# dmMaze/comic-text-detector

Hardware: AMD Instinct MI355X
Metric: pages/sec at 1024x1024 bs=32 (end-to-end detector, device-resident pages) (higher is better)
Workload: dtype f16

## Files before the change

### comic-text-detector_amd/_lib.py

```python
from __future__ import annotations

import ctypes as C
import os
import subprocess

_HERE = os.path.dirname(os.path.abspath(__file__))
LIB_PATH = os.path.join(_HERE, "libctd_hip.so")
SELFTEST_PATH = os.path.join(_HERE, "ctd_selftest")

ABI_VERSION = 8
OK = 0
PREC_F32, PREC_F16, PREC_F32S = 0, 1, 2
ACT = {"none": 0, "silu": 1, "leaky": 2, "relu": 3, "sigmoid": 4}
IN_NCHW_F32, IN_NHWC_U8 = 0, 1
(OP_INPUT, OP_CONV, OP_CONVT, OP_MAXPOOL, OP_AVGPOOL2, OP_DETECT, OP_EXPORT, OP_STEM, OP_SEG_FINAL,
 OP_DB_UP) = range(1, 11)
OUT_MASK, OUT_LINES = 0, 1
REGION_OK, REGION_DEGENERATE, REGION_MAX_SIDE, REGION_TILE = 0, 1, 32766, 1024
REGION_U8, REGION_F16, REGION_F32 = 0, 1, 2
LAYOUT_NCHW, LAYOUT_NHWC = 0, 1


class CtdTensor(C.Structure):
    _fields_ = [("channels", C.c_int32), ("log2_down", C.c_int32), ("dtype", C.c_int32)]
# ... 64 lines not shown
    "ctd_ccl_workspace_bytes": (C.c_size_t, [_i32, _i32, _i32]),
    "ctd_ccl": (_i32, [_vp, _i32, _i32, _i32, _i32, _i32, _vp, _vp, _vp, _i32, _vp, C.c_size_t, _vp]),
    "ctd_ccl_dual": (_i32, [_vp, _i32, _i32, _i32, _i32, _vp, _vp, _vp, _vp, _vp, _vp, _vp, _i32, _vp, C.c_size_t, _vp]),
    "ctd_resize_linear_u8": (_i32, [_vp, _i32, _i32, _i32, _vp, _i32, _i32, _i32, _i32, _vp]),
    "ctd_region_transforms": (_i32, [_vp, _vp, _vp, _vp, _vp, _vp, _i32, C.c_double, _vp, _vp, _vp, _vp]),
    "ctd_warp_regions": (_i32, [_vp, _i32, _vp, _i32, _vp, _vp]),
    "ctd_warp_region_batches": (_i32, [_vp, _i32, _vp, _i32, _vp, _vp, _i32, _i32, _i32, _i32, _vp]),
    "ctd_db_boxes": (_i32, [_vp, _vp, _vp, _i32, _vp, _vp, _i32, _i32, _i32, _i32, C.c_double, _vp, _vp, C.POINTER(_i32)]),
    "ctd_tail_create": (_i32, [C.POINTER(_vp), _i32]),
    "ctd_tail_destroy": (None, [_vp]),
    "ctd_tail_stream": (_vp, [_vp]),
    "ctd_tail_run": (_i32, [_vp, _i32, _i32, _i32, _vp, _i32, _i32, _vp, _vp, _i64, _vp, C.POINTER(CtdTailPage),
                            C.POINTER(CtdTailParams), _vp, _vp, _vp]),
    "ctd_tail_timings": (_i32, [_vp, C.POINTER(C.c_double)]),
    "ctd_tail_refine_paths": (_i32, [_vp, C.POINTER(_i32)]),
    "ctd_tail_db_boxes": (_i32, [_vp, _i32, _i32, _i32, _vp, _i64, _vp, _i32, C.c_double]),
    "ctd_tail_refine": (_i32, [_vp, _i32, C.POINTER(CtdTailPage), _vp, _vp, _vp, _i32, _i32, _vp, _vp]),
    "ctd_tail_page_counts": (_i32, [_vp, _i32, C.POINTER(_i32), C.POINTER(_i32), C.POINTER(_i32), C.POINTER(_i32),
                                    C.POINTER(_i32)]),
    "ctd_tail_page_fetch": (_i32, [_vp, _i32, _vp, _vp, _vp, _vp, _vp, _vp, _vp, _vp]),
    "ctd_tail_batch_counts": (_i32, [_vp, _vp]),
    "ctd_tail_batch_fetch": (_i32, [_vp, _vp, _vp, _vp]),
    "ctd_tail_pack_records": (_i32, [_vp, _i32, _i32, _vp]),
    "ctd_tail_set_threads": (_i32, [_vp, _i32]),
    "ctd_db_boxes_compact": (_i32, [_i32, _i32, _i32, _vp, _vp, _vp, _vp, _vp, _i32, _vp, _vp, _vp, _vp, _vp, _vp, _vp, _vp,
                                    _vp, _i32, C.c_double, _vp, _vp, C.POINTER(_i32)]),
    "ctd_topk_colors": (_i32, [_vp, _vp]),
    "ctd_otsu_from_hist": (_i32, [_vp]),
    "ctd_inrange_bounds": (None, [C.c_double, C.c_double, C.POINTER(_i32), C.POINTER(_i32)]),
    "ctd_group_output": (_i32, [_vp, _vp, _i32, _vp, _i32, _i32, _i32, _vp, _i32, _vp, _i32, _vp, _i32, _vp, _i32,
# ... 70 lines not shown
```

### comic-text-detector_amd/csrc/engine.hip

```cpp
#include <algorithm>
#include <cmath>
#include <cstdio>
#include <cstdlib>
#include <cstring>
#include <string>
#include <vector>

#include "kernels.h"

namespace {

thread_local std::string g_err;

int fail(int code, const std::string& msg) {
  g_err = msg;
  return code;
}

#define HIP_TRY(expr)                                                                              \
  do {                                                                                             \
    hipError_t _e = (expr);                                                                        \
    if (_e != hipSuccess)                                                                          \
      return fail(CTD_ERR_HIP, std::string(#expr) + ": " + hipGetErrorString(_e));                 \
  } while (0)
// ... 1023 lines not shown
}

int ctd_fail_msg(int code, const std::string& msg) { return fail(code, msg); }
extern int g_tail_priority;
extern int g_tail_cus, g_tail_cu_first;
extern long long g_tail_dma_min;
#ifdef CTD_MEASURE_KNOBS
extern int g_tail_skip_pages;
extern int g_tail_ablate;
#endif
extern int g_tail_chain;
extern int g_tail_fused_rounds;
extern long long g_tail_fused_max_pix;
extern int g_tail_lds, g_tail_lds_rcap, g_tw_lds_runs_x10, g_tw_lds_threads;
extern long long g_tail_lds_cls0, g_tail_lds_cls1;
extern long long g_tail_lds_max_bytes;

extern "C" {

const char* ctd_last_error(void) { return g_err.c_str(); }
int32_t ctd_abi_version(void) { return CTD_ABI_VERSION; }

int ctd_device_info(int32_t device, char* name, int32_t* cu_count, int64_t* hbm_bytes) {
  hipDeviceProp_t p;
  HIP_TRY(hipGetDeviceProperties(&p, device));
  if (name) { std::strncpy(name, p.name, 255); name[255] = 0; }
  if (cu_count) *cu_count = p.multiProcessorCount;
  if (hbm_bytes) *hbm_bytes = (int64_t)p.totalGlobalMem;
  int arch = 0;
  const char* g = std::strstr(p.gcnArchName, "gfx");
// ... 145 lines not shown
int ctd_tuning_set(const char* key, int64_t value) {
  const std::string k = key ? key : "";
  if (k == "fuse") g_fuse = (int)value;
  else if (k == "tail_max_blocks") g_tail_max_blocks = (int)std::max<int64_t>(1, value);
  else if (k == "tail_chain") g_tail_chain = (int)value;
  else if (k == "tail_fused_rounds") g_tail_fused_rounds = (int)value;
  else if (k == "tail_fused_max_pix") g_tail_fused_max_pix = value;
  else if (k == "tail_lds") g_tail_lds = (int)value;
  else if (k == "tail_lds_rcap") g_tail_lds_rcap = (int)value;
  else if (k == "tail_lds_max_bytes") g_tail_lds_max_bytes = value;
  else if (k == "tail_lds_runs_x10") g_tw_lds_runs_x10 = (int)std::max<int64_t>(1, value);
  else if (k == "tail_lds_threads") g_tw_lds_threads = (int)value;
  else if (k == "tail_lds_cls0") g_tail_lds_cls0 = value;
  else if (k == "tail_lds_cls1") g_tail_lds_cls1 = value;
  else if (k == "tail_dma_min") g_tail_dma_min = value;
#ifdef CTD_MEASURE_KNOBS
  else if (k == "tail_skip_page_download") g_tail_skip_pages = value != 0;
  else if (k == "tail_ablate") g_tail_ablate = (int)value;
#endif
  else if (k == "tail_priority") g_tail_priority = (int)value;
  else if (k == "tail_cus") g_tail_cus = (int)value;
  else if (k == "tail_cu_first") g_tail_cu_first = (int)value;
  else if (k == "no_reuse") g_no_reuse = (int)value;
  else if (k == "f32_mfma") g_f32_mfma = (int)value;
  else if (k == "split_halo") g_split_halo = (int)value;
  else if (k == "split_halo_min_patches") g_split_halo_min_patches = value;
  else if (k == "fwd_prio") g_fwd_prio = (int)value;
  else if (k == "split_stem") g_split_stem = (int)value;
  else if (k == "split_planes") g_split_planes = (int)value;
  else if (k == "db_up_mfma") g_db_up_mfma = (int)value;
// ... 101 lines not shown
```

### comic-text-detector_amd/csrc/tail.h

```cpp
#pragma once
#include "ctd_common.h"

extern int g_tail_max_blocks;

struct DbcTables {
  int B, H, W, cap, rcap;
  const float* prob;
  long long prob_stride;
  const int* lab;
  const int* n_f;
  const int* n_b;
  const int* st_f;
  const int* st_b;
  const int* first_f;
  const int* first_b;
  int* par_f;
  int* par_b;
  int* off_f;
  int* off_b;
  int* hdr;
  int* row_lo;
  int* row_hi;
  double* sum_f;
  double* sum_b;
  double* ring_sum;
  int* ring_cnt;
};
void launch_dbc(const DbcTables& t, hipStream_t st);

struct TWin {
  const uint8_t* img;
  const uint8_t* mask;
  uint8_t* out;
  int img_w, mask_w, out_w;
  int x1, y1, w, h;
  int mx, my;
  int band0, nband;
};
struct TRule {
  int kind;
  int lo, hi;
};
struct TBand {
// ... 49 lines not shown
```

### comic-text-detector_amd/csrc/tail.hip

```cpp
#include <algorithm>
#include <atomic>
#include <chrono>
#include <mutex>
#include <cmath>
#include <cstring>
#include <string>
#include <thread>
#include <vector>

#include "host_refine.h"
#include "kernels.h"
#include "tail.h"

int ctd_fail_msg(int code, const std::string& msg);
int g_tail_priority = 1;
int g_tail_cus = 0, g_tail_cu_first = 0;

#define T_TRY(expr)                                                                                  \
  do {                                                                                               \
    hipError_t e_ = (expr);                                                                          \
    if (e_ != hipSuccess) return ctd_fail_msg(CTD_ERR_HIP, std::string(#expr) + ": " + hipGetErrorString(e_)); \
  } while (0)

namespace {
// ... 82 lines not shown
  auto work = [&]() {
    for (int i; (i = next.fetch_add(1)) < n;) f(i);
  };
  std::vector<std::thread> th;
  th.reserve(nt - 1);
  for (int k = 1; k < nt; ++k) th.emplace_back(work);
  work();
  for (auto& x : th) x.join();
}

}
int g_tail_chain = 1;
int g_tail_fused_rounds = 1;
long long g_tail_fused_max_pix = 100000;
int g_tail_lds = 1, g_tail_lds_rcap = 0;
long long g_tail_lds_max_bytes = 150 << 10;
long long g_tail_lds_cls0 = 40 << 10, g_tail_lds_cls1 = 80 << 10;
namespace {
struct ChainState {
  std::mutex mu;
  hipEvent_t last = nullptr;
  hipEvent_t ring[16] = {};
  unsigned next = 0;
};
constexpr int kChainDevices = 64;
inline ChainState* chain_state(int device) {
  static ChainState states[kChainDevices];
  return device >= 0 && device < kChainDevices ? &states[device] : nullptr;
}
struct GpuChain {
// ... 81 lines not shown
  if (a.type == hipMemoryTypeHost && a.devicePointer) return a.devicePointer;
  return nullptr;
}

inline double now_ms() {
  return std::chrono::duration<double, std::milli>(std::chrono::steady_clock::now().time_since_epoch()).count();
}

}

struct ctd_tail {
  int device = 0;
  hipStream_t st = nullptr;
  DevBuf d_dets, d_nms_ws, d_lab_f, d_ccl_ws, d_ccl_small, d_dbc_i, d_dbc_d, d_rows, d_pmask, d_refined;
  DevBuf d_wins, d_rules, d_bands, d_hist, d_sums, d_canvas, d_clab, d_cstats, d_cnt, d_merged, d_mlab, d_mstats, d_cnt2, d_small, d_crop;
  DevBuf d_wins_c, d_bands_c, d_lds;
  PinBuf h_dets, h_hdr, h_tab, h_pmask, h_refined, h_hist, h_sums, h_wins, h_rules, h_bands, h_small, h_lab;
  PinBuf h_wins_c, h_bands_c, h_lds;
  int B = 0;
  std::vector<ctd_tail_page> pages;
  std::vector<size_t> poff;
  std::vector<uint8_t*> hmask;
  size_t ptotal = 0;
  std::vector<PageOut> out;
  double ms_stage[10] = {0, 0, 0, 0, 0, 0, 0, 0, 0, 0};
  double ms_db_wait = 0;
  double ms_sub[5] = {0, 0, 0, 0, 0};
  int host_threads = 8;
  int n_lds = 0, n_canvas = 0, n_ovf = 0;
  long long lds_per_block = 64 << 10;
  double ms_lds_wait = 0;
};

namespace {

struct Packed {
  std::vector<int> x, y;
  int W = 0, H = 0;
};
void shelf_pack(const std::vector<int>& w, const std::vector<int>& h, int min_width, Packed& out) {
  const int n = (int)w.size();
  out.x.assign(n, 0);
  out.y.assign(n, 0);
  int cw = min_width;
// ... 392 lines not shown
  const double w0 = now_ms();
  T_TRY(hipStreamSynchronize(st));
  t->ms_sub[3] = now_ms() - w0;
  return CTD_OK;
}

struct DbStage {
  int B = 0, Hn = 0, Wn = 0;
  const float* prob = nullptr;
  long long prob_stride = 0;
  int *lab = nullptr, *n_f = nullptr, *n_b = nullptr, *st_f = nullptr, *st_b = nullptr;
  int *first_f = nullptr, *first_b = nullptr, *par_f = nullptr, *par_b = nullptr, *off_f = nullptr, *off_b = nullptr;
  int *hdr = nullptr, *ring_cnt = nullptr, *row_lo = nullptr, *row_hi = nullptr;
  double *sum_f = nullptr, *sum_b = nullptr, *ring_sum = nullptr;
  int* hhdr = nullptr;
};

int db_enqueue(ctd_tail* t, DbStage& d, int B, int Hn, int Wn, const float* prob_dev, long long prob_stride,
               const uint8_t* bitmap_dev, Batch& pre, Batch& post) {
  hipStream_t st = t->st;
  const size_t hw = (size_t)Hn * Wn;
  const int cap = kCompCap, rcap = kRowCap;
  d.B = B, d.Hn = Hn, d.Wn = Wn, d.prob = prob_dev, d.prob_stride = prob_stride;
  GET(t->d_lab_f, (size_t)B * hw * 4, int, lab);
  GET(t->d_ccl_ws, ccl_workspace_bytes(B, Hn, Wn), uint8_t, ccl_ws);
  const size_t bc = (size_t)B * cap;
  GET(t->d_dbc_i, (2 * (size_t)B + 10 * bc + 6 * bc + 4 * (size_t)B + bc) * 4, int, ti);
  d.lab = lab;
  d.n_f = ti;
  d.n_b = d.n_f + B;
  d.st_f = d.n_b + B;
  d.st_b = d.st_f + 5 * bc;
  d.first_f = d.st_b + 5 * bc;
  d.first_b = d.first_f + bc;
  d.par_f = d.first_b + bc;
  d.par_b = d.par_f + bc;
  d.off_f = d.par_b + bc;
  d.off_b = d.off_f + bc;
  d.hdr = d.off_b + bc;
  d.ring_cnt = d.hdr + 4 * (size_t)B;
  GET(t->d_dbc_d, 3 * bc * 8, double, td);
  d.sum_f = td, d.sum_b = td + bc, d.ring_sum = td + 2 * bc;
  GET(t->d_rows, 2 * (size_t)B * rcap * 4, int, rows);
  d.row_lo = rows, d.row_hi = rows + (size_t)B * rcap;
  pre.fill(td, 0, 3 * bc * 8);
  pre.fill(d.ring_cnt, 0, bc * 4);
  pre.flush();
  launch_ccl_dual(bitmap_dev, B, Hn, Wn, 0, lab, d.n_f, d.n_b, d.st_f, d.st_b, d.first_f, d.first_b, cap, ccl_ws, st);
  DbcTables dt;
  dt.B = B, dt.H = Hn, dt.W = Wn, dt.cap = cap, dt.rcap = rcap;
  dt.prob = prob_dev, dt.prob_stride = prob_stride;
  dt.lab = lab, dt.n_f = d.n_f, dt.n_b = d.n_b, dt.st_f = d.st_f, dt.st_b = d.st_b;
  dt.first_f = d.first_f, dt.first_b = d.first_b, dt.par_f = d.par_f, dt.par_b = d.par_b, dt.off_f = d.off_f;
  dt.off_b = d.off_b, dt.hdr = d.hdr, dt.row_lo = d.row_lo, dt.row_hi = d.row_hi, dt.sum_f = d.sum_f, dt.sum_b = d.sum_b;
  dt.ring_sum = d.ring_sum, dt.ring_cnt = d.ring_cnt;
  launch_dbc(dt, st);
  GET(t->h_hdr, (size_t)B * 4 * 4, int, hhdr);
  d.hhdr = hhdr;
  T_TRY(post.d2h(hhdr, d.hdr, (size_t)B * 16));
// ... 71 lines not shown
    int nbox = 0;
    const int rc = ctd_db_boxes_compact(Wn, Hn, hhdr[4 * b], h_st_f + (size_t)b * nf * 5, h_first_f + (size_t)b * nf,
                                        h_par_f + (size_t)b * nf, h_off_f + (size_t)b * nf, h_sum_f + (size_t)b * nf,
                                        hhdr[4 * b + 1], h_st_b + (size_t)b * nb * 5, h_first_b + (size_t)b * nb,
                                        h_par_b + (size_t)b * nb, h_off_b + (size_t)b * nb, h_sum_b + (size_t)b * nb,
                                        h_ring_sum + (size_t)b * nb, h_ring_cnt + (size_t)b * nb, h_row_lo + (size_t)b * nr,
                                        h_row_hi + (size_t)b * nr, maxc, prm->unclip_ratio, po.db_boxes.data(),
                                        po.db_scores.data(), &nbox);
    if (rc) err = rc;
    po.db_boxes.resize((size_t)nbox * 8);
    po.db_scores.resize(nbox);
  });
  if (err) return ctd_fail_msg(err, "ctd_db_boxes_compact failed");
  std::vector<int16_t> boxes((size_t)std::max(maxc, 1) * 8);
  std::vector<float> scores((size_t)std::max(maxc, 1));
  for (int b = 0; b < B; ++b) {
    if (!hhdr[4 * b + 3]) continue;
    PageOut& po = t->out[b];
    int nbox = 0;
    {
      std::vector<int32_t> lab_host_f(hw), lab_host_b(hw);
      std::vector<float> prob_h(hw);
      int nfb[2];
      T_TRY(hipMemcpyAsync(nfb, d.n_f + b, 4, hipMemcpyDeviceToHost, st));
      T_TRY(hipMemcpyAsync(nfb + 1, d.n_b + b, 4, hipMemcpyDeviceToHost, st));
      T_TRY(hipMemcpyAsync(lab_host_f.data(), d.lab + (size_t)b * hw, hw * 4, hipMemcpyDeviceToHost, st));
      T_TRY(hipMemcpyAsync(prob_h.data(), d.prob + (size_t)b * d.prob_stride, hw * 4, hipMemcpyDeviceToHost, st));
      T_TRY(hipStreamSynchronize(st));
      for (size_t i = 0; i < hw; ++i) {
        const int32_t l = lab_host_f[i];
        lab_host_f[i] = l > 0 ? l : 0;
        lab_host_b[i] = l < 0 ? -l : 0;
      }
      std::vector<int32_t> sf((size_t)nfb[0] * 5), sb((size_t)nfb[1] * 5);
      auto stats_of = [&](const std::vector<int32_t>& lab, std::vector<int32_t>& s, int n) {
        for (int l = 0; l < n; ++l) {
          int32_t* q = s.data() + 5 * (size_t)l;
          q[0] = Wn, q[1] = Hn, q[2] = -1, q[3] = -1, q[4] = 0;
        }
        for (int y = 0; y < Hn; ++y)
          for (int x = 0; x < Wn; ++x) {
// ... 49 lines not shown
  if (hipDeviceGetAttribute(&smem, hipDeviceAttributeMaxSharedMemoryPerBlock, device) == hipSuccess && smem > 0) t->lds_per_block = smem;
  *out = t;
  return CTD_OK;
}

void ctd_tail_destroy(ctd_tail* t) {
  if (!t) return;
  (void)hipSetDevice(t->device);
  if (t->st) {
    (void)hipStreamSynchronize(t->st);
    (void)hipStreamDestroy(t->st);
  }
  DevBuf* dv[] = {&t->d_dets, &t->d_nms_ws, &t->d_lab_f, &t->d_ccl_ws, &t->d_ccl_small, &t->d_dbc_i, &t->d_dbc_d,
                  &t->d_rows, &t->d_pmask, &t->d_refined, &t->d_wins, &t->d_rules, &t->d_bands, &t->d_hist, &t->d_sums,
                  &t->d_canvas, &t->d_clab, &t->d_cstats, &t->d_cnt, &t->d_merged, &t->d_mlab, &t->d_mstats, &t->d_cnt2,
                  &t->d_small, &t->d_crop, &t->d_wins_c, &t->d_bands_c, &t->d_lds};
  for (DevBuf* d : dv) d->release();
  PinBuf* pv[] = {&t->h_dets, &t->h_hdr, &t->h_tab, &t->h_pmask, &t->h_refined, &t->h_hist, &t->h_sums, &t->h_wins,
                  &t->h_rules, &t->h_bands, &t->h_small, &t->h_lab, &t->h_wins_c, &t->h_bands_c, &t->h_lds};
  for (PinBuf* p : pv) p->release();
  delete t;
}

void* ctd_tail_stream(ctd_tail* t) { return t ? (void*)t->st : nullptr; }

static int drained(ctd_tail* t, int rc) {
  if (rc != CTD_OK && t && t->st) (void)hipStreamSynchronize(t->st);
  return rc;
}

static int tail_run_impl(ctd_tail* t, int32_t B, int32_t Hn, int32_t Wn, const float* blks_dev, int32_t rows, int32_t no,
// ... 178 lines not shown
                 const ctd_tail_page* pages, const ctd_tail_params* prm, uint8_t* const* mask_out,
                 uint8_t* const* refined_out, void* ready_event) {
  return drained(t, tail_run_impl(t, B, Hn, Wn, blks_dev, rows, no, mask_u8_dev, prob_dev, prob_stride, bitmap_dev, pages, prm,
                                  mask_out, refined_out, ready_event));
}

int ctd_tail_timings(const ctd_tail* t, double* ms16) {
  if (!t || !ms16) return ctd_fail_msg(CTD_ERR_INVALID, "null argument");
  std::memcpy(ms16, t->ms_stage, sizeof(t->ms_stage));
  ms16[10] = t->ms_db_wait;
  for (int i = 0; i < 5; ++i) ms16[11 + i] = t->ms_sub[i];
  ms16[15] = t->ms_lds_wait;
  return CTD_OK;
}

int ctd_tail_refine_paths(const ctd_tail* t, int32_t* counts3) {
  if (!t || !counts3) return ctd_fail_msg(CTD_ERR_INVALID, "null argument");
  counts3[0] = t->n_lds, counts3[1] = t->n_canvas, counts3[2] = t->n_ovf;
  return CTD_OK;
}

static int tail_db_boxes_impl(ctd_tail* t, int32_t B, int32_t Hn, int32_t Wn, const float* prob_dev, int64_t prob_stride,
                             const uint8_t* bitmap_dev, int32_t max_candidates, double unclip_ratio) {
  if (!t || !prob_dev || !bitmap_dev || B < 1 || Hn < 1 || Wn < 1) return ctd_fail_msg(CTD_ERR_INVALID, "bad arguments");
  T_TRY(hipSetDevice(t->device));
  t->B = B;
  t->out.assign(B, PageOut());
  DbStage db;
  Batch pre(t->st), post(t->st);
  if (int rc = db_enqueue(t, db, B, Hn, Wn, prob_dev, prob_stride, bitmap_dev, pre, post)) return rc;
// ... 144 lines not shown
```

### comic-text-detector_amd/tail.py

```python
from __future__ import annotations

import ctypes as C
import threading
from typing import List, Optional, Sequence, Tuple

import numpy as np
import torch

from . import _lib as L
from .textblock import BLK_DTYPE, BlockList, TextBlock, blocks_from_batch, blocks_from_records


def _pinned_u8(h: int, w: int) -> np.ndarray:
    return torch.empty((h, w), dtype=torch.uint8, pin_memory=True).numpy()


def _pinned_pages(shapes) -> List[np.ndarray]:
    sizes = [h * w for h, w in shapes]
    buf = torch.empty((sum(sizes),), dtype=torch.uint8, pin_memory=True).numpy()
    out, off = [], 0
    for (h, w), n in zip(shapes, sizes):
        out.append(buf[off: off + n].reshape(h, w))
        off += n
    return out
# ... 148 lines not shown
        return out

    def timings(self) -> dict:
        ms = (C.c_double * 16)()
        L.check(self._lib.ctd_tail_timings(self._h, ms), "ctd_tail_timings")
        keys = ("enqueue1", "wait1", "db_tables+geometry", "yolo+group_output", "refine_wait_hist", "refine_wait_xor",
                "refine_host+enqueue", "undetected", "final_wait+copies", "total", "db_table_wait", "enq1_nms+buffers",
                "enq1_labelling+tables", "enq1_mask_copies", "final_wait_only", "refine_wait_merge")
        return {k: round(v, 3) for k, v in zip(keys, ms)}

    def refine_paths(self) -> dict:
        c = (C.c_int32 * 3)()
        L.check(self._lib.ctd_tail_refine_paths(self._h, c), "ctd_tail_refine_paths")
        return {"lds": int(c[0]), "canvas": int(c[1]), "overflow": int(c[2])}

    def db_boxes(self, prob: torch.Tensor, bitmap: torch.Tensor, max_candidates=1000, unclip_ratio=1.5):
        B, Hn, Wn = bitmap.shape
        prob = prob.float().contiguous()
        bitmap = bitmap.contiguous()
        torch.cuda.current_stream(self.device).synchronize()
        L.check(self._lib.ctd_tail_db_boxes(self._h, B, Hn, Wn, prob.data_ptr(), prob.stride(0), bitmap.data_ptr(),
                                            int(max_candidates), float(unclip_ratio)), "ctd_tail_db_boxes")
        boxes, scores = [], []
        for b in range(B):
            nx = C.c_int32()
            L.check(self._lib.ctd_tail_page_counts(self._h, b, None, None, None, C.byref(nx), None), "ctd_tail_page_counts")
            bx = np.empty((nx.value, 4, 2), np.int16)
            sc = np.empty((nx.value,), np.float32)
            L.check(self._lib.ctd_tail_page_fetch(self._h, b, None, None, None, bx.ctypes.data, sc.ctypes.data, None, None,
                                                  None), "ctd_tail_page_fetch")
# ... 91 lines not shown
```

### include/ctd_hip.h

```cpp
#ifndef CTD_HIP_H
#define CTD_HIP_H

#include <stddef.h>
#include <stdint.h>

#ifdef __cplusplus
extern "C" {
#endif

#define CTD_ABI_VERSION 8

#define CTD_OK 0
#define CTD_ERR_INVALID (-1)
#define CTD_ERR_HIP (-2)
#define CTD_ERR_UNSUPPORTED (-3)
#define CTD_ERR_NOMEM (-4)

#define CTD_PREC_F32 0
#define CTD_PREC_F16 1
#define CTD_PREC_F32S 2

#define CTD_ACT_NONE 0
#define CTD_ACT_SILU 1
#define CTD_ACT_LEAKY 2
// ... 154 lines not shown
  int32_t pad_;
} ctd_tail_params;

int ctd_tail_create(ctd_tail** out, int32_t device);
void ctd_tail_destroy(ctd_tail* t);
void* ctd_tail_stream(ctd_tail* t);

int ctd_tail_run(ctd_tail* t, int32_t B, int32_t Hn, int32_t Wn, const float* blks_dev, int32_t rows, int32_t no,
                 const uint8_t* mask_u8_dev, const float* prob_dev, int64_t prob_stride, const uint8_t* bitmap_dev,
                 const ctd_tail_page* pages, const ctd_tail_params* prm, uint8_t* const* mask_out,
                 uint8_t* const* refined_out, void* ready_event);

int ctd_tail_timings(const ctd_tail* t, double* ms);

int ctd_tail_refine_paths(const ctd_tail* t, int32_t* counts3);

int ctd_tail_db_boxes(ctd_tail* t, int32_t B, int32_t Hn, int32_t Wn, const float* prob_dev, int64_t prob_stride,
                      const uint8_t* bitmap_dev, int32_t max_candidates, double unclip_ratio);

int ctd_tail_refine(ctd_tail* t, int32_t n_pages, const ctd_tail_page* pages, const uint8_t* const* masks_host,
                    const int32_t* blk_xyxy, const int32_t* blk_counts, int32_t refine_mode, int32_t keep_undetected_mask,
                    uint8_t* const* mask_out, uint8_t* const* refined_out);

int ctd_tail_page_counts(const ctd_tail* t, int32_t page, int32_t* n_blocks, int32_t* n_lines, int32_t* n_dist,
                         int32_t* n_db_boxes, int32_t* n_yolo);
struct ctd_blk;
int ctd_tail_page_fetch(const ctd_tail* t, int32_t page, struct ctd_blk* blocks, int32_t* lines, double* dist,
                        int16_t* db_boxes, float* db_scores, int32_t* yolo_xyxy, int32_t* yolo_cls, float* yolo_conf);

int ctd_tail_batch_counts(const ctd_tail* t, int32_t* counts);
// ... 57 lines not shown
```

Baseline: 3226.

## Replace pixel-level DB-box labeling with run-length connected components

Adds a run-length-encoded connected-component path for DB box extraction. It bit-packs the bitmap, builds the runs, unions vertically overlapping runs, ranks the roots, and gathers component stats, row extents, probability sums and holes per run instead of per pixel. This is meant to remove the full per-pixel label buffer and the cost of pixel-level CCL in the tail. Pages that overflow a capacity fall back to a per-page dual CCL, which adds code complexity and some extra scan and launch overhead.

```diff
diff --git a/comic-text-detector_amd/_lib.py b/comic-text-detector_amd/_lib.py
--- a/comic-text-detector_amd/_lib.py
+++ b/comic-text-detector_amd/_lib.py
@@ -102,6 +102,7 @@
                             C.POINTER(CtdTailParams), _vp, _vp, _vp]),
     "ctd_tail_timings": (_i32, [_vp, C.POINTER(C.c_double)]),
     "ctd_tail_refine_paths": (_i32, [_vp, C.POINTER(_i32)]),
+    "ctd_tail_db_paths": (_i32, [_vp, C.POINTER(_i32)]),
     "ctd_tail_db_boxes": (_i32, [_vp, _i32, _i32, _i32, _vp, _i64, _vp, _i32, C.c_double]),
     "ctd_tail_refine": (_i32, [_vp, _i32, C.POINTER(CtdTailPage), _vp, _vp, _vp, _i32, _i32, _vp, _vp]),
     "ctd_tail_page_counts": (_i32, [_vp, _i32, C.POINTER(_i32), C.POINTER(_i32), C.POINTER(_i32), C.POINTER(_i32),
diff --git a/comic-text-detector_amd/csrc/engine.hip b/comic-text-detector_amd/csrc/engine.hip
--- a/comic-text-detector_amd/csrc/engine.hip
+++ b/comic-text-detector_amd/csrc/engine.hip
@@ -1061,6 +1061,7 @@
 extern long long g_tail_fused_max_pix;
 extern int g_tail_lds, g_tail_lds_rcap, g_tw_lds_runs_x10, g_tw_lds_threads;
 extern long long g_tail_lds_cls0, g_tail_lds_cls1;
+extern int g_tail_db_runs, g_tail_db_run_cap;
 extern long long g_tail_lds_max_bytes;
 
 extern "C" {
@@ -1236,6 +1237,8 @@
   else if (k == "tail_lds_cls0") g_tail_lds_cls0 = value;
   else if (k == "tail_lds_cls1") g_tail_lds_cls1 = value;
   else if (k == "tail_dma_min") g_tail_dma_min = value;
+  else if (k == "tail_db_runs") g_tail_db_runs = (int)value;
+  else if (k == "tail_db_run_cap") g_tail_db_run_cap = (int)std::max<int64_t>(0, value);
 #ifdef CTD_MEASURE_KNOBS
   else if (k == "tail_skip_page_download") g_tail_skip_pages = value != 0;
   else if (k == "tail_ablate") g_tail_ablate = (int)value;
diff --git a/comic-text-detector_amd/csrc/kernels_dbruns.hip b/comic-text-detector_amd/csrc/kernels_dbruns.hip
--- /dev/null
+++ b/comic-text-detector_amd/csrc/kernels_dbruns.hip
@@ -0,0 +1,485 @@
+#include <hip/amd_detail/amd_hip_unsafe_atomics.h>
+
+#include <algorithm>
+
+#include "tail.h"
+
+namespace {
+
+__device__ __forceinline__ int uf_load(const int* parent, int x) {
+  return __hip_atomic_load(parent + x, __ATOMIC_RELAXED, __HIP_MEMORY_SCOPE_AGENT);
+}
+__device__ __forceinline__ int uf_find(const int* parent, int x) {
+  int p = uf_load(parent, x);
+  while (p != x) {
+    x = p;
+    p = uf_load(parent, x);
+  }
+  return x;
+}
+__device__ __forceinline__ void uf_union(int* parent, int a, int b) {
+  while (true) {
+    a = uf_find(parent, a);
+    b = uf_find(parent, b);
+    if (a == b) return;
+    if (a > b) { const int t = a; a = b; b = t; }
+    const int old = atomicMin(parent + b, a);
+    if (old == b) return;
+    b = old;
+  }
+}
+
+__device__ __forceinline__ int block_excl_scan(int v, int* sh, int* total) {
+  const int lane = threadIdx.x & 63, w = threadIdx.x >> 6;
+  int incl = v;
+  for (int off = 1; off < 64; off <<= 1) {
+    const int u = __shfl_up(incl, off);
+    if (lane >= off) incl += u;
+  }
+  if (lane == 63) sh[w] = incl;
+  __syncthreads();
+  int base = 0;
+  for (int i = 0; i < w; ++i) base += sh[i];
+  *total = sh[0] + sh[1] + sh[2] + sh[3];
+  __syncthreads();
+  return base + incl - v;
+}
+
+__device__ __forceinline__ unsigned nz4(unsigned v) {
+  const unsigned m = ((((v & 0x7f7f7f7fu) + 0x7f7f7f7fu) | v) & 0x80808080u) >> 7;
+  return (m | (m >> 7) | (m >> 14) | (m >> 21)) & 0xfu;
+}
+
+__device__ __forceinline__ int run_of(const DbrTables& t, int b, int y, int x) {
+  const int g = y * t.ww + (x >> 5);
+  const size_t pg = (size_t)b * t.nw + g;
+  return t.blk[b * t.nblk + (g >> 8)] + (int)t.wbase[pg] + __popc(t.starts[pg] & (0xffffffffu >> (31 - (x & 31)))) - 1;
+}
+
+__global__ __launch_bounds__(256) void dbr_pack_kernel(DbrTables t) {
+  __shared__ int sh[4];
+  const int b = blockIdx.y;
+  const uint8_t* img = t.img + (size_t)b * t.H * t.W;
+  const bool vec = (t.W & 15) == 0 && ((uintptr_t)t.img & 15) == 0;
+  for (int k = blockIdx.x; k < t.nblk; k += gridDim.x) {
+    const int g = k * 256 + (int)threadIdx.x;
+    unsigned s = 0;
+    if (g < t.nw) {
+      const int y = g / t.ww, wi = g - y * t.ww;
+      const int x0 = wi * 32, nv = min(32, t.W - x0);
+      const uint8_t* p = img + (size_t)y * t.W + x0;
+      unsigned w = 0;
+      if (vec && nv == 32) {
+        const uint4 a = ((const uint4*)p)[0], c = ((const uint4*)p)[1];
+        w = nz4(a.x) | (nz4(a.y) << 4) | (nz4(a.z) << 8) | (nz4(a.w) << 12) | (nz4(c.x) << 16) | (nz4(c.y) << 20) |
+            (nz4(c.z) << 24) | (nz4(c.w) << 28);
+      } else {
+        for (int i = 0; i < nv; ++i) w |= (p[i] > 0 ? 1u : 0u) << i;
+      }
+      const unsigned prev = wi > 0 ? (p[-1] > 0 ? 1u : 0u) : (~w & 1u);
+      s = (w ^ ((w << 1) | prev)) & (nv == 32 ? 0xffffffffu : ((1u << nv) - 1u));
+      t.starts[(size_t)b * t.nw + g] = s;
+    }
+    int total;
+    const int e = block_excl_scan(__popc(s), sh, &total);
+    if (g < t.nw) t.wbase[(size_t)b * t.nw + g] = (unsigned short)e;
+    if (threadIdx.x == 0) t.blk[b * t.nblk + k] = total;
+  }
+}
+
+__global__ __launch_bounds__(256) void dbr_scan_words_kernel(DbrTables t) {
+  __shared__ int sh[4];
+  const int b = blockIdx.x;
+  int* a = t.blk + b * t.nblk;
+  int carry = 0;
+  for (int base = 0; base < t.nblk; base += 256) {
+    const int i = base + (int)threadIdx.x;
+    const int v = i < t.nblk ? a[i] : 0;
+    int total;
+    const int e = block_excl_scan(v, sh, &total);
+    if (i < t.nblk) a[i] = carry + e;
+    carry += total;
+  }
+  if (threadIdx.x == 0) {
+    t.n_runs[b] = carry;
+    t.nholes[b] = 0;
+    if (carry <= t.run_cap) t.rinfo[(size_t)b * (t.run_cap + 1) + carry] = (t.H * t.W) << 1;
+  }
+}
+
+__global__ __launch_bounds__(256) void dbr_runs_kernel(DbrTables t) {
+  const int b = blockIdx.y;
+  if (t.n_runs[b] > t.run_cap) return;
+  const uint8_t* img = t.img + (size_t)b * t.H * t.W;
+  int* rinfo = t.rinfo + (size_t)b * (t.run_cap + 1);
+  int* parent = t.parent + (size_t)b * t.run_cap;
+  for (int g = blockIdx.x * 256 + (int)threadIdx.x; g < t.nw; g += gridDim.x * 256) {
+    unsigned s = t.starts[(size_t)b * t.nw + g];
+    if (!s) continue;
+    const int y = g / t.ww, wi = g - y * t.ww;
+    const int p0 = y * t.W + wi * 32;
+    int r = t.blk[b * t.nblk + (g >> 8)] + (int)t.wbase[(size_t)b * t.nw + g];
+    int c = img[p0 + __ffs((int)s) - 1] > 0 ? 1 : 0;
+    while (s) {
+      const int bit = __ffs((int)s) - 1;
+      s &= s - 1;
+      rinfo[r] = ((p0 + bit) << 1) | c;
+      parent[r] = r;
+      ++r, c ^= 1;
+    }
+  }
+}
+
+struct RunGeo {
+  int p, c, y, x0, x1;
+};
+__device__ __forceinline__ RunGeo run_geo(const int* rinfo, int r, int W) {
+  RunGeo q;
+  const int ri = rinfo[r];
+  q.p = ri >> 1, q.c = ri & 1;
+  q.y = q.p / W;
+  q.x0 = q.p - q.y * W;
+  q.x1 = min(rinfo[r + 1] >> 1, (q.y + 1) * W) - 1 - q.y * W;
+  return q;
+}
+
+__global__ __launch_bounds__(256) void dbr_link_kernel(DbrTables t) {
+  const int b = blockIdx.y;
+  const int nr = t.n_runs[b];
+  if (nr > t.run_cap) return;
+  const int* rinfo = t.rinfo + (size_t)b * (t.run_cap + 1);
+  int* parent = t.parent + (size_t)b * t.run_cap;
+  for (int r = blockIdx.x * 256 + (int)threadIdx.x; r < nr; r += gridDim.x * 256) {
+    const RunGeo q = run_geo(rinfo, r, t.W);
+    if (q.y == 0) continue;
+    const int lo = q.c ? max(q.x0 - 1, 0) : q.x0, hi = q.c ? min(q.x1 + 1, t.W - 1) : q.x1;
+    const int last = (q.y - 1) * t.W + hi;
+    int u = run_of(t, b, q.y - 1, lo);
+    if ((rinfo[u] & 1) != q.c) ++u;
+    for (; u < r; u += 2) {
+      if ((rinfo[u] >> 1) > last) break;
+      uf_union(parent, r, u);
+    }
+  }
+}
+
+__global__ __launch_bounds__(256) void dbr_flatten_kernel(DbrTables t) {
+  const int b = blockIdx.y;
+  const int nr = t.n_runs[b];
+  if (nr > t.run_cap) return;
+  const int* rinfo = t.rinfo + (size_t)b * (t.run_cap + 1);
+  int* parent = t.parent + (size_t)b * t.run_cap;
+  __shared__ int cnt[2];
+  for (int k = blockIdx.x; k * 256 < nr; k += gridDim.x) {
+    if (threadIdx.x < 2) cnt[threadIdx.x] = 0;
+    __syncthreads();
+    const int r = k * 256 + (int)threadIdx.x;
+    bool root = false;
+    int c = 0;
+    if (r < nr) {
+      const int rt = uf_find(parent, r);
+      root = rt == r;
+      c = rinfo[r] & 1;
+      if (!root) __hip_atomic_store(parent + r, rt, __ATOMIC_RELAXED, __HIP_MEMORY_SCOPE_AGENT);
+    }
+    const int nf = __popcll(__ballot(root && c)), nb = __popcll(__ballot(root && !c));
+    if ((threadIdx.x & 63) == 0) {
+      if (nf) atomicAdd(&cnt[1], nf);
+      if (nb) atomicAdd(&cnt[0], nb);
+    }
+    __syncthreads();
+    if (threadIdx.x < 2) t.ccnt[((size_t)b * 2 + threadIdx.x) * t.nchunk + k] = cnt[threadIdx.x];
+    __syncthreads();
+  }
+}
+
+__global__ __launch_bounds__(256) void dbr_scan_roots_kernel(DbrTables t) {
+  __shared__ int sh[4];
+  const int b = blockIdx.x >> 1, c = blockIdx.x & 1;
+  const int nr = t.n_runs[b];
+  int* out = c ? t.n_f : t.n_b;
+  if (nr > t.run_cap) {
+    if (threadIdx.x == 0) out[b] = 0;
+    return;
+  }
+  const int n = (nr + 255) >> 8;
+  int* a = t.ccnt + ((size_t)b * 2 + c) * t.nchunk;
+  int carry = 0;
+  for (int base = 0; base < n; base += 256) {
+    const int i = base + (int)threadIdx.x;
+    const int v = i < n ? a[i] : 0;
+    int total;
+    const int e = block_excl_scan(v, sh, &total);
+    if (i < n) a[i] = carry + e;
+    carry += total;
+  }
+  if (threadIdx.x == 0) out[b] = carry;
+}
+
+__global__ __launch_bounds__(256) void dbr_rank_kernel(DbrTables t) {
+  __shared__ int sh[4];
+  const int b = blockIdx.y;
+  const int nr = t.n_runs[b];
+  if (nr > t.run_cap) return;
+  const int* rinfo = t.rinfo + (size_t)b * (t.run_cap + 1);
+  const int* parent = t.parent + (size_t)b * t.run_cap;
+  int* comp = t.comp + (size_t)b * t.run_cap;
+  const size_t cb = (size_t)b * t.cap;
+  for (int k = blockIdx.x; k * 256 < nr; k += gridDim.x) {
+    const int r = k * 256 + (int)threadIdx.x;
+    const bool root = r < nr && parent[r] == r;
+    const int ri = root ? rinfo[r] : 0;
+    const int c = ri & 1;
+    int total;
+    const int e = block_excl_scan(root ? (c ? 1 : 1 << 16) : 0, sh, &total);
+    if (!root) continue;
+    const int id = t.ccnt[((size_t)b * 2 + c) * t.nchunk + k] + (c ? (e & 0xffff) : (e >> 16)) + 1;
+    comp[r] = c ? id : -id;
+    if (id > t.cap) continue;
+    const size_t l = cb + id - 1;
+    int* s = (c ? t.st_f : t.st_b) + l * 5;
+    s[0] = t.W, s[1] = t.H, s[2] = -1, s[3] = -1, s[4] = 0;
+    if (c) {
+      t.first_f[l] = ri >> 1, t.par_f[l] = r, t.sum_f[l] = 0.0;
+    } else {
+      t.first_b[l] = ri >> 1, t.par_b[l] = r, t.sum_b[l] = 0.0, t.ring_sum[l] = 0.0, t.ring_cnt[l] = 0;
+    }
+  }
+}
+
+__device__ __forceinline__ int wave_min(int v) {
+  for (int off = 32; off > 0; off >>= 1) v = min(v, __shfl_xor(v, off));
+  return v;
+}
+__device__ __forceinline__ int wave_max(int v) {
+  for (int off = 32; off > 0; off >>= 1) v = max(v, __shfl_xor(v, off));
+  return v;
+}
+__device__ __forceinline__ int wave_sum(int v) {
+  for (int off = 32; off > 0; off >>= 1) v += __shfl_xor(v, off);
+  return v;
+}
+
+__global__ __launch_bounds__(256) void dbr_stats_kernel(DbrTables t) {
+  const int b = blockIdx.y;
+  const int nr = t.n_runs[b];
+  if (nr > t.run_cap) return;
+  const int* rinfo = t.rinfo + (size_t)b * (t.run_cap + 1);
+  const int* parent = t.parent + (size_t)b * t.run_cap;
+  int* comp = t.comp + (size_t)b * t.run_cap;
+  const size_t cb = (size_t)b * t.cap;
+  const int lane = threadIdx.x & 63;
+  for (int base = blockIdx.x * 256; base < nr; base += gridDim.x * 256) {
+    const int r = base + (int)threadIdx.x;
+    const bool live = r < nr;
+    int id = 0;
+    RunGeo q{0, 0, 0, 0, 0};
+    if (live) {
+      const int rt = parent[r];
+      id = comp[rt];
+      if (rt != r) comp[r] = id;
+      q = run_geo(rinfo, r, t.W);
+    }
+    const int mag = id > 0 ? id : -id;
+    bool on = live && mag <= t.cap;
+    for (int round = 0; round < 2; ++round) {
+      const unsigned long long m = __ballot(on);
+      if (!m) break;
+      const int leader = __ffsll((long long)m) - 1;
+      const int v = __shfl(id, leader);
+      const bool same = on && id == v;
+      if (__popcll(__ballot(same)) < 4) break;
+      const int a0 = wave_min(same ? q.x0 : 0x7fffffff), a1 = wave_min(same ? q.y : 0x7fffffff);
+      const int a2 = wave_max(same ? q.x1 : -1), a3 = wave_max(same ? q.y : -1);
+      const int a4 = wave_sum(same ? q.x1 - q.x0 + 1 : 0);
+      if (lane == leader) {
+        int* s = (v > 0 ? t.st_f : t.st_b) + (cb + (v > 0 ? v : -v) - 1) * 5;
+        atomicMin(s + 0, a0), atomicMin(s + 1, a1), atomicMax(s + 2, a2), atomicMax(s + 3, a3), atomicAdd(s + 4, a4);
+      }
+      on = on && !same;
+    }
+    if (on) {
+      int* s = (id > 0 ? t.st_f : t.st_b) + (cb + mag - 1) * 5;
+      atomicMin(s + 0, q.x0), atomicMin(s + 1, q.y), atomicMax(s + 2, q.x1), atomicMax(s + 3, q.y), atomicAdd(s + 4, q.x1 - q.x0 + 1);
+    }
+  }
+}
+
+__global__ __launch_bounds__(256) void dbr_prep_kernel(DbrTables t) {
+  const int b = blockIdx.y;
+  const int nf = min(t.n_f[b], t.cap), nb = min(t.n_b[b], t.cap);
+  const int* comp = t.comp + (size_t)b * t.run_cap;
+  for (int l = blockIdx.x * 256 + (int)threadIdx.x; l < max(nf, nb); l += gridDim.x * 256) {
+    const size_t r = (size_t)b * t.cap + l;
+    if (l < nf) {
+      int* s = t.st_f + r * 5;
+      s[2] -= s[0] - 1, s[3] -= s[1] - 1;
+      const int run = t.par_f[r];
+      t.par_f[r] = (t.first_f[r] % t.W) > 0 ? max(-comp[run - 1], 0) : 0;
+      t.off_f[r] = s[3];
+    }
+    if (l < nb) {
+      int* s = t.st_b + r * 5;
+      s[2] -= s[0] - 1, s[3] -= s[1] - 1;
+      const bool hole = s[0] > 0 && s[1] > 0 && s[0] + s[2] < t.W && s[1] + s[3] < t.H;
+      const int run = t.par_b[r];
+      t.par_b[r] = hole ? max(comp[run - 1], 0) : 0;
+      t.off_b[r] = hole ? s[3] + 2 : 0;
+      if (hole) atomicAdd(t.nholes + b, 1);
+    }
+  }
+}
+
+__global__ __launch_bounds__(256) void dbr_scan_rows_kernel(DbrTables t) {
+  __shared__ int sh[4];
+  const int b = blockIdx.x;
+  const int nf = min(t.n_f[b], t.cap), nb = min(t.n_b[b], t.cap);
+  int carry = 0;
+  for (int pass = 0; pass < 2; ++pass) {
+    int* a = (pass ? t.off_b : t.off_f) + (size_t)b * t.cap;
+    const int n = pass ? nb : nf;
+    for (int base = 0; base < n; base += 256) {
+      const int i = base + (int)threadIdx.x;
+      const int v = i < n ? a[i] : 0;
+      int total;
+      const int e = block_excl_scan(v, sh, &total);
+      if (i < n) a[i] = carry + e;
+      carry += total;
+    }
+  }
+  if (threadIdx.x == 0) {
+    int* h = t.hdr + b * 4;
+    h[0] = nf, h[1] = nb, h[2] = carry;
+    h[3] = ((t.n_f[b] > t.cap || t.n_b[b] > t.cap || carry > t.rcap) ? 1 : 0) | (t.n_runs[b] > t.run_cap ? 2 : 0);
+  }
+}
+
+__global__ __launch_bounds__(256) void dbr_rows_init_kernel(DbrTables t) {
+  const int b = blockIdx.y;
+  const int n = min(t.hdr[b * 4 + 2], t.rcap);
+  if (t.hdr[b * 4 + 3]) return;
+  const size_t rb = (size_t)b * t.rcap;
+  for (int r = blockIdx.x * 256 + (int)threadIdx.x; r < n; r += gridDim.x * 256) t.row_lo[rb + r] = 0x7fffffff, t.row_hi[rb + r] = -1;
+}
+
+__global__ __launch_bounds__(256) void dbr_accum_kernel(DbrTables t) {
+  const int b = blockIdx.y;
+  const int nr = t.n_runs[b];
+  if (t.hdr[b * 4 + 3]) return;
+  const int* rinfo = t.rinfo + (size_t)b * (t.run_cap + 1);
+  const int* comp = t.comp + (size_t)b * t.run_cap;
+  const float* prob = t.prob + (long long)b * t.prob_stride;
+  const size_t cb = (size_t)b * t.cap, rb = (size_t)b * t.rcap;
+  const bool holes = t.nholes[b] > 0;
+  const int W = t.W, H = t.H;
+  for (int r = blockIdx.x * 256 + (int)threadIdx.x; r < nr; r += gridDim.x * 256) {
+    const RunGeo q = run_geo(rinfo, r, W);
+    const int id = comp[r];
+    if (!q.c) {
+      const int lb = -id;
+      if (t.par_b[cb + lb - 1] <= 0) continue;
+      double s = 0.0;
+      for (int x = q.x0; x <= q.x1; ++x) s += (double)prob[q.p + x - q.x0];
+      unsafeAtomicAdd(t.sum_b + cb + lb - 1, s);
+      continue;
+    }
+    const int lf = id;
+    double s = 0.0;
+    for (int x = q.x0; x <= q.x1; ++x) s += (double)prob[q.p + x - q.x0];
+    unsafeAtomicAdd(t.sum_f + cb + lf - 1, s);
+    const int row = t.off_f[cb + lf - 1] + (q.y - t.st_f[(cb + lf - 1) * 5 + 1]);
+    atomicMin(t.row_lo + rb + row, q.x0);
+    atomicMax(t.row_hi + rb + row, q.x1);
+    if (!holes) continue;
+    const int hl = q.x0 > 0 ? -comp[r - 1] : 0, hr = q.x1 + 1 < W ? -comp[r + 1] : 0;
+    int qu = 0, eu = 0x7fffffff, hu = 0, qd = 0, ed = 0x7fffffff, hd = 0;
+    if (q.y > 0) {
+      qu = run_of(t, b, q.y - 1, q.x0);
+      eu = (rinfo[qu + 1] >> 1) - (q.y - 1) * W;
+      hu = -comp[qu];
+    }
+    if (q.y + 1 < H) {
+      qd = run_of(t, b, q.y + 1, q.x0);
+      ed = (rinfo[qd + 1] >> 1) - (q.y + 1) * W;
+      hd = -comp[qd];
+    }
+    for (int x = q.x0; x <= q.x1; ++x) {
+      while (x >= eu) {
+        ++qu;
+        eu = (rinfo[qu + 1] >> 1) - (q.y - 1) * W;
+        hu = -comp[qu];
+      }
+      while (x >= ed) {
+        ++qd;
+        ed = (rinfo[qd + 1] >> 1) - (q.y + 1) * W;
+        hd = -comp[qd];
+      }
+      const int hbs[4] = {x == q.x0 ? hl : 0, x == q.x1 ? hr : 0, hu, hd};
+      int seen[4];
+      int ns = 0;
+      for (int k = 0; k < 4; ++k) {
+        const int hb = hbs[k];
+        if (hb <= 0 || t.par_b[cb + hb - 1] != lf) continue;
+        bool dup = false;
+        for (int j = 0; j < ns; ++j) dup |= seen[j] == hb;
+        if (dup) continue;
+        seen[ns++] = hb;
+        unsafeAtomicAdd(t.ring_sum + cb + hb - 1, (double)prob[q.p + x - q.x0]);
+        atomicAdd(t.ring_cnt + cb + hb - 1, 1);
+        const int rw = t.off_b[cb + hb - 1] + (q.y - (t.st_b[(cb + hb - 1) * 5 + 1] - 1));
+        atomicMin(t.row_lo + rb + rw, x);
+        atomicMax(t.row_hi + rb + rw, x);
+      }
+    }
+  }
+}
+
+inline size_t up256(size_t v) { return (v + 255) / 256 * 256; }
+
+}
+
+int dbr_run_cap(int H, int W) {
+  const long long hw = (long long)H * W;
+  return (int)std::min<long long>(hw, std::max<long long>(hw / 4, 1 << 16));
+}
+
+size_t dbr_workspace_bytes(int B, int H, int W, int run_cap) {
+  const size_t nw = (size_t)H * ((W + 31) / 32), nblk = (nw + 255) / 256, nchunk = ((size_t)run_cap + 255) / 256;
+  return up256((size_t)B * nw * 4) + up256((size_t)B * nw * 2) + up256((size_t)B * nblk * 4) + 2 * up256((size_t)B * 4) +
+         up256((size_t)B * ((size_t)run_cap + 1) * 4) + 2 * up256((size_t)B * run_cap * 4) + up256((size_t)B * 2 * nchunk * 4);
+}
+
+void launch_dbr(DbrTables t, void* ws, hipStream_t st) {
+  t.ww = (t.W + 31) / 32, t.nw = t.H * t.ww, t.nblk = (t.nw + 255) / 256, t.nchunk = (t.run_cap + 255) / 256;
+  const size_t B = (size_t)t.B;
+  char* p = (char*)ws;
+  auto take = [&](size_t bytes) {
+    char* q = p;
+    p += up256(bytes);
+    return q;
+  };
+  t.starts = (unsigned*)take(B * t.nw * 4);
+  t.wbase = (unsigned short*)take(B * t.nw * 2);
+  t.blk = (int*)take(B * t.nblk * 4);
+  t.n_runs = (int*)take(B * 4);
+  t.nholes = (int*)take(B * 4);
+  t.rinfo = (int*)take(B * ((size_t)t.run_cap + 1) * 4);
+  t.parent = (int*)take(B * t.run_cap * 4);
+  t.comp = (int*)take(B * t.run_cap * 4);
+  t.ccnt = (int*)take(B * 2 * t.nchunk * 4);
+  const int per_page = std::max(1, g_tail_max_blocks / std::max(1, t.B));
+  auto grid = [&](int items) { return dim3(std::max(1, std::min((items + 255) / 256, per_page)), t.B); };
+  const dim3 blk(256);
+  hipLaunchKernelGGL(dbr_pack_kernel, grid(t.nw), blk, 0, st, t);
+  hipLaunchKernelGGL(dbr_scan_words_kernel, dim3(t.B), blk, 0, st, t);
+  hipLaunchKernelGGL(dbr_runs_kernel, grid(t.nw), blk, 0, st, t);
+  hipLaunchKernelGGL(dbr_link_kernel, grid(t.run_cap), blk, 0, st, t);
+  hipLaunchKernelGGL(dbr_flatten_kernel, grid(t.run_cap), blk, 0, st, t);
+  hipLaunchKernelGGL(dbr_scan_roots_kernel, dim3(2 * t.B), blk, 0, st, t);
+  hipLaunchKernelGGL(dbr_rank_kernel, grid(t.run_cap), blk, 0, st, t);
+  hipLaunchKernelGGL(dbr_stats_kernel, grid(t.run_cap), blk, 0, st, t);
+  hipLaunchKernelGGL(dbr_prep_kernel, grid(t.cap), blk, 0, st, t);
+  hipLaunchKernelGGL(dbr_scan_rows_kernel, dim3(t.B), blk, 0, st, t);
+  hipLaunchKernelGGL(dbr_rows_init_kernel, grid(t.rcap), blk, 0, st, t);
+  hipLaunchKernelGGL(dbr_accum_kernel, grid(t.run_cap), blk, 0, st, t);
+}
diff --git a/comic-text-detector_amd/csrc/tail.h b/comic-text-detector_amd/csrc/tail.h
--- a/comic-text-detector_amd/csrc/tail.h
+++ b/comic-text-detector_amd/csrc/tail.h
@@ -27,6 +27,29 @@
   int* ring_cnt;
 };
 void launch_dbc(const DbcTables& t, hipStream_t st);
+
+struct DbrTables {
+  int B, H, W, cap, rcap;
+  int run_cap;
+  const uint8_t* img;
+  const float* prob;
+  long long prob_stride;
+  int *n_f, *n_b, *st_f, *st_b, *first_f, *first_b, *par_f, *par_b, *off_f, *off_b, *hdr, *row_lo, *row_hi, *ring_cnt;
+  double *sum_f, *sum_b, *ring_sum;
+  int ww, nw, nblk, nchunk;
+  unsigned* starts;
+  unsigned short* wbase;
+  int* blk;
+  int* n_runs;
+  int* nholes;
+  int* rinfo;
+  int* parent;
+  int* comp;
+  int* ccnt;
+};
+int dbr_run_cap(int H, int W);
+size_t dbr_workspace_bytes(int B, int H, int W, int run_cap);
+void launch_dbr(DbrTables t, void* ws, hipStream_t st);
 
 struct TWin {
   const uint8_t* img;
diff --git a/comic-text-detector_amd/csrc/tail.hip b/comic-text-detector_amd/csrc/tail.hip
--- a/comic-text-detector_amd/csrc/tail.hip
+++ b/comic-text-detector_amd/csrc/tail.hip
@@ -120,6 +120,7 @@
 int g_tail_fused_rounds = 1;
 long long g_tail_fused_max_pix = 100000;
 int g_tail_lds = 1, g_tail_lds_rcap = 0;
+int g_tail_db_runs = 1, g_tail_db_run_cap = 0;
 long long g_tail_lds_max_bytes = 150 << 10;
 long long g_tail_lds_cls0 = 40 << 10, g_tail_lds_cls1 = 80 << 10;
 namespace {
@@ -231,7 +232,7 @@
   hipStream_t st = nullptr;
   DevBuf d_dets, d_nms_ws, d_lab_f, d_ccl_ws, d_ccl_small, d_dbc_i, d_dbc_d, d_rows, d_pmask, d_refined;
   DevBuf d_wins, d_rules, d_bands, d_hist, d_sums, d_canvas, d_clab, d_cstats, d_cnt, d_merged, d_mlab, d_mstats, d_cnt2, d_small, d_crop;
-  DevBuf d_wins_c, d_bands_c, d_lds;
+  DevBuf d_wins_c, d_bands_c, d_lds, d_dbr;
   PinBuf h_dets, h_hdr, h_tab, h_pmask, h_refined, h_hist, h_sums, h_wins, h_rules, h_bands, h_small, h_lab;
   PinBuf h_wins_c, h_bands_c, h_lds;
   int B = 0;
@@ -245,6 +246,7 @@
   double ms_sub[5] = {0, 0, 0, 0, 0};
   int host_threads = 8;
   int n_lds = 0, n_canvas = 0, n_ovf = 0;
+  int n_db_runs = 0, n_db_label = 0, n_db_rovf = 0;
   long long lds_per_block = 64 << 10;
   double ms_lds_wait = 0;
 };
@@ -667,6 +669,8 @@
   int *hdr = nullptr, *ring_cnt = nullptr, *row_lo = nullptr, *row_hi = nullptr;
   double *sum_f = nullptr, *sum_b = nullptr, *ring_sum = nullptr;
   int* hhdr = nullptr;
+  bool runs = false;
+  const uint8_t* bitmap = nullptr;
 };
 
 int db_enqueue(ctd_tail* t, DbStage& d, int B, int Hn, int Wn, const float* prob_dev, long long prob_stride,
@@ -675,11 +679,9 @@
   const size_t hw = (size_t)Hn * Wn;
   const int cap = kCompCap, rcap = kRowCap;
   d.B = B, d.Hn = Hn, d.Wn = Wn, d.prob = prob_dev, d.prob_stride = prob_stride;
-  GET(t->d_lab_f, (size_t)B * hw * 4, int, lab);
-  GET(t->d_ccl_ws, ccl_workspace_bytes(B, Hn, Wn), uint8_t, ccl_ws);
+  d.runs = g_tail_db_runs != 0, d.bitmap = bitmap_dev;
   const size_t bc = (size_t)B * cap;
   GET(t->d_dbc_i, (2 * (size_t)B + 10 * bc + 6 * bc + 4 * (size_t)B + bc) * 4, int, ti);
-  d.lab = lab;
   d.n_f = ti;
   d.n_b = d.n_f + B;
   d.st_f = d.n_b + B;
@@ -696,6 +698,27 @@
   d.sum_f = td, d.sum_b = td + bc, d.ring_sum = td + 2 * bc;
   GET(t->d_rows, 2 * (size_t)B * rcap * 4, int, rows);
   d.row_lo = rows, d.row_hi = rows + (size_t)B * rcap;
+  if (d.runs) {
+    pre.flush();
+    DbrTables rt;
+    rt.B = B, rt.H = Hn, rt.W = Wn, rt.cap = cap, rt.rcap = rcap;
+    rt.run_cap = dbr_run_cap(Hn, Wn);
+    if (g_tail_db_run_cap > 0) rt.run_cap = std::min(rt.run_cap, g_tail_db_run_cap);
+    rt.img = bitmap_dev, rt.prob = prob_dev, rt.prob_stride = prob_stride;
+    rt.n_f = d.n_f, rt.n_b = d.n_b, rt.st_f = d.st_f, rt.st_b = d.st_b, rt.first_f = d.first_f, rt.first_b = d.first_b;
+    rt.par_f = d.par_f, rt.par_b = d.par_b, rt.off_f = d.off_f, rt.off_b = d.off_b, rt.hdr = d.hdr, rt.row_lo = d.row_lo;
+    rt.row_hi = d.row_hi, rt.ring_cnt = d.ring_cnt, rt.sum_f = d.sum_f, rt.sum_b = d.sum_b, rt.ring_sum = d.ring_sum;
+    GET(t->d_dbr, dbr_workspace_bytes(B, Hn, Wn, rt.run_cap), uint8_t, dbr_ws);
+    launch_dbr(rt, dbr_ws, st);
+    GET(t->h_hdr, (size_t)B * 4 * 4, int, hhdr);
+    d.hhdr = hhdr;
+    T_TRY(post.d2h(hhdr, d.hdr, (size_t)B * 16));
+    T_TRY(hipGetLastError());
+    return CTD_OK;
+  }
+  GET(t->d_lab_f, (size_t)B * hw * 4, int, lab);
+  GET(t->d_ccl_ws, ccl_workspace_bytes(B, Hn, Wn), uint8_t, ccl_ws);
+  d.lab = lab;
   pre.fill(td, 0, 3 * bc * 8);
   pre.fill(d.ring_cnt, 0, bc * 4);
   pre.flush();
@@ -797,17 +820,33 @@
   if (err) return ctd_fail_msg(err, "ctd_db_boxes_compact failed");
   std::vector<int16_t> boxes((size_t)std::max(maxc, 1) * 8);
   std::vector<float> scores((size_t)std::max(maxc, 1));
+  t->n_db_runs = t->n_db_label = t->n_db_rovf = 0;
+  for (int b = 0; b < B; ++b) {
+    if (d.runs && !hhdr[4 * b + 3]) ++t->n_db_runs;
+    else ++t->n_db_label;
+    if (d.runs && (hhdr[4 * b + 3] & 2)) ++t->n_db_rovf;
+  }
   for (int b = 0; b < B; ++b) {
     if (!hhdr[4 * b + 3]) continue;
     PageOut& po = t->out[b];
     int nbox = 0;
+    const int* lab_b = d.lab + (d.runs ? 0 : (size_t)b * hw);
+    if (d.runs) {
+      GET(t->d_lab_f, hw * 4, int, lab1);
+      GET(t->d_ccl_ws, ccl_workspace_bytes(1, Hn, Wn), uint8_t, ws1);
+      const size_t cb = (size_t)b * cap;
+      launch_ccl_dual(d.bitmap + (size_t)b * hw, 1, Hn, Wn, 0, lab1, d.n_f + b, d.n_b + b, d.st_f + cb * 5, d.st_b + cb * 5,
+                      d.first_f + cb, d.first_b + cb, cap, ws1, st);
+      T_TRY(hipGetLastError());
+      lab_b = lab1;
+    }
     {
       std::vector<int32_t> lab_host_f(hw), lab_host_b(hw);
       std::vector<float> prob_h(hw);
       int nfb[2];
       T_TRY(hipMemcpyAsync(nfb, d.n_f + b, 4, hipMemcpyDeviceToHost, st));
       T_TRY(hipMemcpyAsync(nfb + 1, d.n_b + b, 4, hipMemcpyDeviceToHost, st));
-      T_TRY(hipMemcpyAsync(lab_host_f.data(), d.lab + (size_t)b * hw, hw * 4, hipMemcpyDeviceToHost, st));
+      T_TRY(hipMemcpyAsync(lab_host_f.data(), lab_b, hw * 4, hipMemcpyDeviceToHost, st));
       T_TRY(hipMemcpyAsync(prob_h.data(), d.prob + (size_t)b * d.prob_stride, hw * 4, hipMemcpyDeviceToHost, st));
       T_TRY(hipStreamSynchronize(st));
       for (size_t i = 0; i < hw; ++i) {
@@ -887,7 +926,7 @@
   DevBuf* dv[] = {&t->d_dets, &t->d_nms_ws, &t->d_lab_f, &t->d_ccl_ws, &t->d_ccl_small, &t->d_dbc_i, &t->d_dbc_d,
                   &t->d_rows, &t->d_pmask, &t->d_refined, &t->d_wins, &t->d_rules, &t->d_bands, &t->d_hist, &t->d_sums,
                   &t->d_canvas, &t->d_clab, &t->d_cstats, &t->d_cnt, &t->d_merged, &t->d_mlab, &t->d_mstats, &t->d_cnt2,
-                  &t->d_small, &t->d_crop, &t->d_wins_c, &t->d_bands_c, &t->d_lds};
+                  &t->d_small, &t->d_crop, &t->d_wins_c, &t->d_bands_c, &t->d_lds, &t->d_dbr};
   for (DevBuf* d : dv) d->release();
   PinBuf* pv[] = {&t->h_dets, &t->h_hdr, &t->h_tab, &t->h_pmask, &t->h_refined, &t->h_hist, &t->h_sums, &t->h_wins,
                   &t->h_rules, &t->h_bands, &t->h_small, &t->h_lab, &t->h_wins_c, &t->h_bands_c, &t->h_lds};
@@ -1096,6 +1135,12 @@
   return CTD_OK;
 }
 
+int ctd_tail_db_paths(const ctd_tail* t, int32_t* counts3) {
+  if (!t || !counts3) return ctd_fail_msg(CTD_ERR_INVALID, "null argument");
+  counts3[0] = t->n_db_runs, counts3[1] = t->n_db_label, counts3[2] = t->n_db_rovf;
+  return CTD_OK;
+}
+
 int ctd_tail_refine_paths(const ctd_tail* t, int32_t* counts3) {
   if (!t || !counts3) return ctd_fail_msg(CTD_ERR_INVALID, "null argument");
   counts3[0] = t->n_lds, counts3[1] = t->n_canvas, counts3[2] = t->n_ovf;
diff --git a/comic-text-detector_amd/tail.py b/comic-text-detector_amd/tail.py
--- a/comic-text-detector_amd/tail.py
+++ b/comic-text-detector_amd/tail.py
@@ -186,6 +186,11 @@
         L.check(self._lib.ctd_tail_refine_paths(self._h, c), "ctd_tail_refine_paths")
         return {"lds": int(c[0]), "canvas": int(c[1]), "overflow": int(c[2])}
 
+    def db_paths(self) -> dict:
+        c = (C.c_int32 * 3)()
+        L.check(self._lib.ctd_tail_db_paths(self._h, c), "ctd_tail_db_paths")
+        return {"runs": int(c[0]), "label": int(c[1]), "overflow": int(c[2])}
+
     def db_boxes(self, prob: torch.Tensor, bitmap: torch.Tensor, max_candidates=1000, unclip_ratio=1.5):
         B, Hn, Wn = bitmap.shape
         prob = prob.float().contiguous()
diff --git a/include/ctd_hip.h b/include/ctd_hip.h
--- a/include/ctd_hip.h
+++ b/include/ctd_hip.h
@@ -192,6 +192,8 @@
 int ctd_tail_timings(const ctd_tail* t, double* ms);
 
 int ctd_tail_refine_paths(const ctd_tail* t, int32_t* counts3);
+
+int ctd_tail_db_paths(const ctd_tail* t, int32_t* counts3);
 
 int ctd_tail_db_boxes(ctd_tail* t, int32_t B, int32_t Hn, int32_t Wn, const float* prob_dev, int64_t prob_stride,
                       const uint8_t* bitmap_dev, int32_t max_candidates, double unclip_ratio);
```

Result: slower. 1588 (-50.8%).
